# ipl-uw/ZeDO-Release

Hardware: AMD Instinct MI355X
Metric: poses/sec (1000-step sampler, H=50) (higher is better)
Workload: dtype f32; 1 GPU; BASELINE configs[2] (3DPW pw3d_test, H=50, 1000 steps): N=1015 poses/GPU x H=50 hypotheses, IPO 500 it (17 joints) + 1000 OIL steps + P1/P2 min-over-hypotheses selection; random-init ScoreModelFC_Adv weights, synthetic detections; settings=pw3d, rows_per_gpu=50750, poses_total=1015

## Files before the change

zedo-release_amd/csrc/zedo_gemm.hip:

```cpp
#include "zedo_internal.h"
#include "zedo_tile.h"

#include <atomic>
#include <cstdlib>

#ifdef ZEDO_UBENCH
#include "../../tools/ubench/zedo_tile_hooks.inc"
#else
#define TL_MARK(var)
#define TL_FLUSH(t0, t1, t2)
#endif

namespace zedo {

template <int BM, int BN, int WM, int WN, int EPI, int NBUF = 2, int BK = 32, int SCHED = 0, int KSKIP = 0, int KQ = 1>
__device__ __forceinline__ void layer_tile(const LayerArgs &a, const int m0, const int n0, const int out_m0) {
    constexpr int NW = WM * WN;
    constexpr int CPR = BK / 4;
    constexpr int RPD = 64 / CPR;
    constexpr int KG = BK / 8;
    static_assert(BK == 32 || BK == 16, "BK");
    constexpr int TM = BM / WM, TN = BN / WN;
    constexpr int TJ = TM / 32, TI = TN / 32;
    constexpr int IA = BN / RPD / NW, IB = BM / RPD / NW;
    constexpr int IPW = IA + IB;
    static_assert(TM % 32 == 0 && TN % 32 == 0 && IA >= 1 && IB >= 1 && (BN / RPD) % NW == 0 && (BM / RPD) % NW == 0, "tile");
    static_assert(NBUF >= 2 && (NBUF - 1) * IPW <= 63, "ring depth vs the 6-bit vmcnt");

    extern __shared__ __attribute__((aligned(16))) float smem[];
    float *As = smem;
    float *Bs = smem + NBUF * BN * BK;
    float *Ps = smem + layer_tile_lds(BM, BN, WM, NBUF, BK) / sizeof(float) - 3 * BN;

    const int tid = threadIdx.x;
    const int lane = tid & 63;
    const int wid = __builtin_amdgcn_readfirstlane(tid >> 6);
    const int wm = wid / WN, wn = wid % WN;
    const int li = lane & 31, kh = lane >> 5;

    const int drow = lane / CPR, dpos = lane % CPR;
    const int dswz = (BK == 32) ? (drow & 7) : ((drow >> 2) & 3);
    const char *Wbase = reinterpret_cast<const char *>(a.W + (size_t)(n0 + wid * IA * RPD) * a.ldw);
    const char *Xbase = reinterpret_cast<const char *>(a.X + (size_t)(m0 + wid * IB * RPD) * a.ldx);
    const unsigned wlane = (unsigned)(drow * a.ldw + (dpos ^ dswz) * 4) * 4u;
    const unsigned xlane = (unsigned)(drow * a.ldx + (dpos ^ dswz) * 4) * 4u;
    const unsigned lds0 = (unsigned)(size_t)(__attribute__((address_space(3))) float *)smem;
    auto dma_one = [&](int kt, int buf, int p) {
        if (p < IA)
            dma16(Wbase + (size_t)kt * (BK * 4) + (size_t)p * (RPD * 4) * a.ldw, wlane,
                  lds0 + (unsigned)(((buf * BN + (wid * IA + p) * RPD) * BK) * 4));
        else
            dma16(Xbase + (size_t)kt * (BK * 4) + (size_t)(p - IA) * (RPD * 4) * a.ldx, xlane,
                  lds0 + (unsigned)(((NBUF * BN + buf * BM + (wid * IB + (p - IA)) * RPD) * BK) * 4));
    };
    auto dma = [&](int kt, int buf) {
#pragma unroll
        for (int p = 0; p < IPW; ++p) dma_one(kt, buf, p);
    };

    const int fswz = (BK == 32) ? (li & 7) : ((li >> 2) & 3);
    int foff[KG];
#pragma unroll
    for (int kg = 0; kg < KG; ++kg) foff[kg] = ((2 * kg + kh) ^ fswz) * 4;
    const float *Ab0 = As + (wn * TN + li) * BK;
    const float *Bb0 = Bs + (wm * TM + li) * BK;
    f32x4 fa0[TI], fb0[TJ], fa1[TI], fb1[TJ];
    auto fread = [&](f32x4(&fa)[TI], f32x4(&fb)[TJ], int buf, int kg) {
#pragma unroll
        for (int i = 0; i < TI; ++i) fa[i] = *reinterpret_cast<const f32x4 *>(Ab0 + (buf * BN + i * 32) * BK + foff[kg]);
#pragma unroll
        for (int j = 0; j < TJ; ++j) fb[j] = *reinterpret_cast<const f32x4 *>(Bb0 + (buf * BM + j * 32) * BK + foff[kg]);
    };
    f32x16 acc[TI][TJ];
#pragma unroll
    for (int i = 0; i < TI; ++i)
#pragma unroll
        for (int j = 0; j < TJ; ++j)
#pragma unroll
            for (int e = 0; e < 16; ++e) acc[i][j][e] = 0.0f;
    auto mma = [&](const f32x4(&fa)[TI], const f32x4(&fb)[TJ]) {
#pragma unroll
        for (int e = 0; e < 4; ++e)
#pragma unroll
            for (int i = 0; i < TI; ++i)
#pragma unroll
                for (int j = 0; j < TJ; ++j)
                    acc[i][j] = __builtin_amdgcn_mfma_f32_32x32x2f32(fa[i][e], fb[j][e], acc[i][j], 0, 0, 0);
    };
    constexpr int H1 = (IPW + 1) / 2, H2 = IPW - H1;
    auto mma_dma = [&](const f32x4(&fa)[TI], const f32x4(&fb)[TJ], int kt, int buf, int p0, int cnt) {
#pragma unroll
        for (int e = 0; e < 4; ++e) {
#pragma unroll
            for (int q = 0; q < 4; ++q)
                if (q < cnt && q * 4 / cnt == e) {
                    dma_one(kt, buf, p0 + q);
                    __builtin_amdgcn_sched_barrier(0);
                }
#pragma unroll
            for (int i = 0; i < TI; ++i)
#pragma unroll
                for (int j = 0; j < TJ; ++j)
                    acc[i][j] = __builtin_amdgcn_mfma_f32_32x32x2f32(fa[i][e], fb[j][e], acc[i][j], 0, 0, 0);
            __builtin_amdgcn_sched_barrier(0);
        }
    };
    static_assert(SCHED >= 0 && SCHED <= 3, "SCHED: bit 0 = pinned reads, bit 1 = spread DMA");
    static_assert(!(SCHED & 2) || H1 <= 4, "spread DMA: at most 4 instructions per MFMA group");

    TL_MARK(tl0)
    if (EPI != EPI_PARTIAL && tid < BN / 4) {
        *reinterpret_cast<f32x4 *>(Ps + tid * 4) = *reinterpret_cast<const f32x4 *>(a.bias + n0 + tid * 4);
        if constexpr (EPI == EPI_GN_SILU || EPI == EPI_GN_SILU_RES) {
            *reinterpret_cast<f32x4 *>(Ps + BN + tid * 4) = *reinterpret_cast<const f32x4 *>(a.gamma + n0 + tid * 4);
            *reinterpret_cast<f32x4 *>(Ps + 2 * BN + tid * 4) = *reinterpret_cast<const f32x4 *>(a.beta + n0 + tid * 4);
        }
    }
    const int KT = a.K / BK;
    f32x16 qsum[KQ > 1 ? TI : 1][KQ > 1 ? TJ : 1];
    const int KTQ = KT / KQ;
#pragma unroll
    for (int t = 0; t < NBUF; ++t) dma(min(t, KT - 1), t);
    asm volatile("s_waitcnt vmcnt(%0)" ::"n"((NBUF - 1) * IPW) : "memory");
    __syncthreads();
    fread(fa0, fb0, 0, 0);
    TL_MARK(tl1)
    for (int kt0 = 0; kt0 < KT; kt0 += NBUF) {
#pragma unroll
      for (int buf = 0; buf < NBUF; ++buf) {
        const int kt = kt0 + buf;
        const int nxt = (buf + 1 == NBUF) ? 0 : buf + 1;
        const int prv = (buf == 0) ? NBUF - 1 : buf - 1;
        fread(fa1, fb1, buf, 1);
        if constexpr (SCHED & 1) __builtin_amdgcn_sched_barrier(0);
        if constexpr (SCHED & 2) mma_dma(fa0, fb0, min(kt - 1 + NBUF, KT - 1), prv, H1, H2);
        else mma(fa0, fb0);
        if constexpr (KG == 4) {
            fread(fa0, fb0, buf, 2);
            if constexpr (SCHED & 1) __builtin_amdgcn_sched_barrier(0);
            mma(fa1, fb1);
            if constexpr (SCHED & 1) __builtin_amdgcn_sched_barrier(0);
            fread(fa1, fb1, buf, 3);
            if constexpr (SCHED & 1) __builtin_amdgcn_sched_barrier(0);
            mma(fa0, fb0);
        }
        const bool skip_last = KSKIP == 1 && KG == 4 && buf == NBUF - 1;
        asm volatile("s_waitcnt vmcnt(%0)" ::"n"((NBUF - 2) * IPW) : "memory");
        __syncthreads();
        if (skip_last) {
        } else if constexpr (SCHED & 2) {
            fread(fa0, fb0, nxt, 0);
            __builtin_amdgcn_sched_barrier(0);
            mma_dma(fa1, fb1, min(kt + NBUF, KT - 1), buf, 0, H1);
        } else {
            dma(min(kt + NBUF, KT - 1), buf);
            fread(fa0, fb0, nxt, 0);
            if constexpr (SCHED & 1) __builtin_amdgcn_sched_barrier(0);
            mma(fa1, fb1);
            if constexpr (SCHED & 1) __builtin_amdgcn_sched_barrier(0);
        }
      }
      if constexpr (KQ > 1) {
          if ((kt0 + NBUF) % KTQ == 0) {
              const bool first = (kt0 + NBUF == KTQ);
#pragma unroll
              for (int i = 0; i < TI; ++i)
#pragma unroll
                  for (int j = 0; j < TJ; ++j)
#pragma unroll
                      for (int e = 0; e < 16; ++e) {
                          qsum[i][j][e] = first ? acc[i][j][e] : qsum[i][j][e] + acc[i][j][e];
                          acc[i][j][e] = 0.0f;
                      }
          }
      }
    }
    if constexpr (KQ > 1) {
#pragma unroll
        for (int i = 0; i < TI; ++i)
#pragma unroll
            for (int j = 0; j < TJ; ++j) acc[i][j] = qsum[i][j];
    }
    asm volatile("s_waitcnt vmcnt(0)" ::: "memory");
    __syncthreads();
    TL_MARK(tl2)

    {
        constexpr int NT = NW * 64;
        constexpr int SR = WM * 32;
        constexpr int CPRW = BN / 4;
        constexpr int RPI = 64 / CPRW;
        static_assert(CPRW <= 64 && 64 % CPRW == 0 && SR % (RPI * NW) == 0 && (SR * CPRW) % NT == 0, "stage shape");
        constexpr bool HAS_RES = (EPI == EPI_GN_SILU_RES || EPI == EPI_SDE);
        float *S = smem;
        float *obase = a.out + (size_t)out_m0 * a.ldo + n0;
#pragma unroll
        for (int j = 0; j < TJ; ++j) {
            if constexpr (HAS_RES) {
                constexpr int NI = SR / RPI / NW;
#pragma unroll
                for (int p = 0; p < NI; ++p) {
                    const int idx = wid * NI + p;
                    const int sr = idx * RPI + lane / CPRW, pos = lane % CPRW;
                    const int grow = (sr >> 5) * TM + j * 32 + (sr & 31);
                    __builtin_amdgcn_global_load_lds(
                        (const __attribute__((address_space(1))) void *)(reinterpret_cast<const char *>(obase) +
                                                                         ((unsigned)grow * (unsigned)a.ldo + (unsigned)((pos ^ (sr & 7)) * 4)) * 4u),
                        (__attribute__((address_space(3))) void *)(S + idx * RPI * BN), 16, 0, 0);
                }
                asm volatile("s_waitcnt vmcnt(0)" ::: "memory");
                __syncthreads();
            }
#pragma unroll
            for (int i = 0; i < TI; ++i) {
                float o[16];
                f32x4 b4[4], ga[4], be[4];
                const float *pc = Ps + wn * TN + i * 32 + 4 * kh;
#pragma unroll
                for (int g = 0; g < 4; ++g) {
                    b4[g] = *reinterpret_cast<const f32x4 *>(pc + 8 * g);
                    if constexpr (EPI == EPI_GN_SILU || EPI == EPI_GN_SILU_RES) {
                        ga[g] = *reinterpret_cast<const f32x4 *>(pc + BN + 8 * g);
                        be[g] = *reinterpret_cast<const f32x4 *>(pc + 2 * BN + 8 * g);
                    }
                }
                epilogue_values<EPI>(acc[i][j], b4, ga, be, a.sde_c, o);
                float *srow = S + (wm * 32 + li) * BN;
#pragma unroll
                for (int g = 0; g < 4; ++g) {
                    const int c = (wn * TN + i * 32 + 8 * g + 4 * kh) >> 2;
                    f32x4 *slot = reinterpret_cast<f32x4 *>(srow + ((c ^ (li & 7)) << 2));
                    f32x4 v = {o[4 * g], o[4 * g + 1], o[4 * g + 2], o[4 * g + 3]};
                    if constexpr (EPI == EPI_GN_SILU_RES) {
                        const f32x4 h = *slot;
#pragma unroll
                        for (int e = 0; e < 4; ++e) v[e] += h[e];
                    } else if constexpr (EPI == EPI_SDE) {
                        const f32x4 x = *slot;
#pragma unroll
                        for (int e = 0; e < 4; ++e) v[e] = __builtin_fmaf(a.sde_a, x[e], v[e]);
                    }
                    *slot = v;
                }
            }
            __syncthreads();
            if constexpr (EPI == EPI_SDE && BN == XLD) {
                if (a.rp.geom != nullptr) {
                    if (tid < SR) {
                        const int sr = tid;
                        const int b = m0 + (sr >> 5) * TM + j * 32 + (sr & 31);
                        if (b < a.rp.B) ZEDO_REPROJ_STAGED_ROW(17, S + sr * BN, sr & 7, b, a.rp);
                    }
                    __syncthreads();
                }
            }
#pragma unroll
            for (int pass = 0; pass < SR * CPRW / NT; ++pass) {
                const int qi = pass * NT + tid;
                const int sr = qi / CPRW, c = qi % CPRW;
                const f32x4 v = *reinterpret_cast<const f32x4 *>(S + sr * BN + ((c ^ (sr & 7)) << 2));
                const int grow = (sr >> 5) * TM + j * 32 + (sr & 31);
                const unsigned off = ((unsigned)grow * (unsigned)a.ldo + (unsigned)(c * 4)) * 4u;
                *reinterpret_cast<f32x4 *>(reinterpret_cast<char *>(obase) + off) = v;
            }
            if (j + 1 < TJ) __syncthreads();
        }
    }
    TL_FLUSH(tl0, tl1, tl2)
}

template <int BM, int BN, int WM, int WN, int EPI, int NBUF = 2, int BK = 32, int SCHED = 0, int KSKIP = 0, int KQ = 1>
__device__ __forceinline__ void layer_body(const LayerArgs &a, const int bid, const int nwg) {
    const int lid = xcd_tile(bid, nwg);
    const int ncol = a.N / BN;
    if constexpr (EPI == EPI_PARTIAL) {
        LayerArgs b = a;
        const int tile = lid >> 2, q = lid & 3;
        b.X = a.X + (size_t)q * a.K;
        b.W = a.W + (size_t)q * a.K;
        layer_tile<BM, BN, WM, WN, EPI, NBUF, BK, SCHED, KSKIP, 1>(b, tile * BM, 0, lid * BM);
        return;
    }
    layer_tile<BM, BN, WM, WN, EPI, NBUF, BK, SCHED, KSKIP, KQ>(a, (lid / ncol) * BM, (lid % ncol) * BN, (lid / ncol) * BM);
}

template <int BM, int BN, int WM, int WN, int EPI, int NBUF = 2, int BK = 32, int SCHED = 0, int WPE = 1, int KSKIP = 0, int KQ = 1>
__global__ __launch_bounds__(WM *WN * 64, WPE) void layer_kernel(LayerArgs a) {
    layer_body<BM, BN, WM, WN, EPI, NBUF, BK, SCHED, KSKIP, KQ>(a, blockIdx.x, gridDim.x);
}

constexpr int SCHED_BIG = 3, SCHED_SMALL = 0, SCHED_THIN = 3, SCHED_BK16 = 1;

constexpr int PAIR_BK = 16, PLAIN_WGS = 3, PLAIN_WPE = 2;
template <int EPI, int W8>
__global__ __launch_bounds__(W8 ? 512 : 256, W8 ? 6 : PLAIN_WGS) void layer_pair_kernel(LayerArgs big, LayerArgs small, int nbig) {
    const ClockProbe probe(big.clk != nullptr && blockIdx.x == 0 && threadIdx.x == 0);
    if constexpr (W8) {
        if ((int)blockIdx.x < nbig) layer_body<128, 128, 2, 4, EPI, 2, PAIR_BK, SCHED_BK16>(big, blockIdx.x, nbig);
        else layer_body<64, 128, 2, 4, EPI, 2, 32, SCHED_SMALL>(small, (int)blockIdx.x - nbig, (int)gridDim.x - nbig);
    } else {
        if ((int)blockIdx.x < nbig) layer_body<128, 128, 2, 2, EPI, 2, PAIR_BK, SCHED_BK16>(big, blockIdx.x, nbig);
        else layer_body<64, 64, 2, 2, EPI, 2, 32, SCHED_SMALL>(small, (int)blockIdx.x - nbig, (int)gridDim.x - nbig);
    }
    probe.stop(big.clk);
}


template <int EPI, int W8>
static hipError_t launch_pair(const LayerArgs &big, const LayerArgs &small, hipStream_t st) {
    constexpr int SM = 64, SN = W8 ? 128 : 64;
    constexpr size_t lds_big = layer_tile_lds(128, 128, 2, 2, PAIR_BK), lds_small = layer_tile_lds(SM, SN, 2, 2, 32);
    constexpr size_t lds = lds_big > lds_small ? lds_big : lds_small;
    if (big.Mp % 128 || small.Mp % SM || big.N % 128 || big.K % 64) return hipErrorInvalidValue;
    auto kern = layer_pair_kernel<EPI, W8>;
    static std::atomic<bool> attr_done[MAX_DEVICES];
    if (hipError_t e = allow_lds(reinterpret_cast<const void *>(kern), lds, attr_done); e != hipSuccess) return e;
    const int nbig = (big.Mp / 128) * (big.N / 128), nsmall = (small.Mp / SM) * (small.N / SN);
    hipLaunchKernelGGL(kern, dim3(nbig + nsmall), dim3(W8 ? 512 : 256), lds, st, big, small, nbig);
    return hipGetLastError();
}

template <int BM, int BN, int WM, int WN, int EPI, int NBUF = 2, int BK = 32, int SCHED = 0, int WPE = 1, int KSKIP = 0, int KQ = 1>
static hipError_t launch_cfg(const LayerArgs &a, hipStream_t st) {
    constexpr size_t lds = layer_tile_lds(BM, BN, WM, NBUF, BK);
    if (a.Mp <= 0 || a.Mp % BM || a.N % BN || a.K % (BK * NBUF * KQ)) return hipErrorInvalidValue;
    if (KSKIP && a.K != BK * NBUF) return hipErrorInvalidValue;
    auto kern = layer_kernel<BM, BN, WM, WN, EPI, NBUF, BK, SCHED, WPE, KSKIP, KQ>;
    static std::atomic<bool> attr_done[MAX_DEVICES];
    if (hipError_t e = allow_lds(reinterpret_cast<const void *>(kern), lds, attr_done); e != hipSuccess) return e;
    const int nwg = (a.Mp / BM) * (a.N / BN) * (EPI == EPI_PARTIAL ? 4 : 1);
    hipLaunchKernelGGL(kern, dim3(nwg), dim3(WM * WN * 64), lds, st, a);
    return hipGetLastError();
}

static LayerArgs rows_of(const LayerArgs &a, int row0, int rows) {
    LayerArgs b = a;
    b.X = a.X + (size_t)row0 * a.ldx;
    b.out = a.out + (size_t)row0 * a.ldo;
    b.Mp = rows;
    return b;
}

template <int EPI>
static hipError_t launch_small(const LayerArgs &a, hipStream_t st) {
    const int ncol = a.N / 128, cus = num_cus();
    if (a.Mp % 64 == 0 && (a.Mp / 64) * (a.N / 64) <= cus)
        return launch_cfg<64, 64, 2, 2, EPI, 4, 32, SCHED_THIN & 1>(a, st);
    if (a.Mp % 32 == 0 && (a.Mp / 32) * ncol <= cus) return launch_cfg<32, 128, 1, 4, EPI, 4, 32, SCHED_THIN & 1>(a, st);
    auto cost = [&](int bm, int slots_per_cu, double tile_us) {
        if (a.Mp % bm) return 1e30;
        const long tiles = (long)(a.Mp / bm) * ncol;
        const long rounds = (tiles + (long)cus * slots_per_cu - 1) / ((long)cus * slots_per_cu);
        return rounds * 6.0 + (double)((tiles + cus - 1) / cus) * tile_us;
    };
    const double kdepth = a.K / 1024.0;
    const double c32 = cost(32, 3, 14.5 * kdepth), c64 = cost(64, 3, 28.2 * kdepth), c128 = cost(128, 2, 55.1 * kdepth);
    if (c32 <= c64 && c32 <= c128) return launch_cfg<32, 128, 1, 4, EPI, 2, 32, SCHED_THIN>(a, st);
    if (c64 <= c128) return launch_cfg<64, 128, 2, 4, EPI, 2, 32, SCHED_THIN>(a, st);
    return launch_cfg<128, 128, 2, 2, EPI, 2, 32, SCHED_BIG, PLAIN_WPE>(a, st);
}

template <int EPI>
static hipError_t launch_wide(const LayerArgs &a, hipStream_t st) {
    if (a.K <= 64) {
        if (a.K == 64 && a.kzero8) return launch_cfg<64, 128, 2, 4, EPI, 2, 32, SCHED_THIN, 1, 1>(a, st);
        return launch_cfg<64, 128, 2, 4, EPI, 2, 32, SCHED_THIN>(a, st);
    }
    constexpr int WG_PER_CU = 3;
    constexpr int W8 = (EPI == EPI_GN_SILU_RES) ? 1 : 0;
    const int per_round = num_cus() * WG_PER_CU * 128 / (a.N / 128);
    int rows_big = (a.Mp / per_round) * per_round;
    if (rows_big == 0) {
        const int one_each = num_cus() * 128 / (a.N / 128);
        const int mix_big = (a.Mp / one_each) * one_each;
        constexpr int SMR = (W8 ? 64 : 32);
        if (mix_big > 0 && a.Mp > mix_big && (a.Mp - mix_big) % SMR == 0) {
            const double kd = a.K / 1024.0;
            const long small_tiles = (long)((a.Mp - mix_big) / SMR) * (a.N / 128);
            const double est_mix = (mix_big / one_each) * 55.1 * kd + (double)((small_tiles + num_cus() - 1) / num_cus()) * (W8 ? 28.2 : 13.9) * kd + 6.0;
            auto single = [&](int bm, int slots, double t) {
                if (a.Mp % bm) return 1e30;
                const long tiles = (long)(a.Mp / bm) * (a.N / 128);
                return (double)((tiles + (long)num_cus() * slots - 1) / ((long)num_cus() * slots)) * 6.0 + (double)((tiles + num_cus() - 1) / num_cus()) * t * kd;
            };
            const double est_single = fmin(fmin(single(32, 3, 14.5), single(64, 3, 28.2)), single(128, 2, 55.1));
            if (est_mix < est_single) rows_big = mix_big;
        }
    }
    const int rows_small = a.Mp - rows_big;
    if (rows_small > 0 && rows_big > 0) {
        if (W8 && rows_small >= 1536) return launch_pair<EPI, W8>(rows_of(a, 0, rows_big), rows_of(a, rows_big, rows_small), st);
        return launch_pair<EPI, 0>(rows_of(a, 0, rows_big), rows_of(a, rows_big, rows_small), st);
    }
    if (rows_big > 0) return launch_pair<EPI, W8>(rows_of(a, 0, rows_big), rows_of(a, rows_big, 0), st);
    return launch_small<EPI>(a, st);
}

hipError_t launch_layer(const LayerArgs &a, int epilogue, hipStream_t st) {
    if (a.N == XLD) {
        if (epilogue != EPI_SDE && epilogue != EPI_BIAS) return hipErrorInvalidValue;
        if (a.K % (4 * 32 * 4)) return hipErrorInvalidValue;
        if (a.Mp <= POST_SPLIT_ROWS && a.Mp % 32 == 0 && a.scratch) {
            LayerArgs p = a;
            p.K = a.K / 4; p.out = a.scratch; p.ldo = XLD;
            if (hipError_t e = launch_cfg<32, 64, 1, 2, EPI_PARTIAL, 4, 32, SCHED_THIN>(p, st); e != hipSuccess) return e;
            const bool sde = epilogue == EPI_SDE;
            return launch_post_reduce(sde ? a.out : nullptr, a.scratch, a.bias, a.sde_a, a.sde_c, sde ? 1 : 0, sde ? nullptr : a.out,
                                      sde ? a.rp : ReprojArgs{}, a.Mp, st);
        }
        const bool small = a.Mp <= 8192 && a.Mp % 32 == 0;
        switch (epilogue) {
            case EPI_SDE: return small ? launch_cfg<32, 64, 1, 2, EPI_SDE, 4, 32, SCHED_THIN, 1, 0, 4>(a, st) : launch_cfg<64, 64, 2, 2, EPI_SDE, 4, 32, SCHED_THIN, 1, 0, 4>(a, st);
            case EPI_BIAS: return small ? launch_cfg<32, 64, 1, 2, EPI_BIAS, 4, 32, SCHED_THIN, 1, 0, 4>(a, st) : launch_cfg<64, 64, 2, 2, EPI_BIAS, 4, 32, SCHED_THIN, 1, 0, 4>(a, st);
        }
        return hipErrorInvalidValue;
    }
    if (a.N % 128) return hipErrorInvalidValue;
    switch (epilogue) {
        case EPI_GN_SILU: return launch_wide<EPI_GN_SILU>(a, st);
        case EPI_GN_SILU_RES: return launch_wide<EPI_GN_SILU_RES>(a, st);
        case EPI_BIAS: return launch_wide<EPI_BIAS>(a, st);
        case EPI_BIAS_SILU: return launch_wide<EPI_BIAS_SILU>(a, st);
    }
    return hipErrorInvalidValue;
}

__global__ __launch_bounds__(256) void mfma_probe_kernel(float *out, int iters, long long *clk) {
    f32x16 acc[4];
    for (int i = 0; i < 4; ++i) for (int e = 0; e < 16; ++e) acc[i][e] = 0.f;
    const float a = threadIdx.x * 1e-3f, b = blockIdx.x * 1e-3f + 1.0f;
    long long t0 = 0, w0 = 0;
    if (threadIdx.x == 0 && blockIdx.x == 0) { t0 = clock64(); w0 = wall_clock64(); }
    for (int it = 0; it < iters; ++it) {
#pragma unroll
        for (int u = 0; u < 4; ++u)
#pragma unroll
            for (int i = 0; i < 4; ++i) acc[i] = __builtin_amdgcn_mfma_f32_32x32x2f32(a, b, acc[i], 0, 0, 0);
    }
    if (threadIdx.x == 0 && blockIdx.x == 0) { clk[0] = clock64() - t0; clk[1] = wall_clock64() - w0; }
    float s = 0;
    for (int i = 0; i < 4; ++i) for (int e = 0; e < 16; ++e) s += acc[i][e];
    out[blockIdx.x * 256 + threadIdx.x] = s;
}

__global__ __launch_bounds__(256) void mfma16_probe_kernel(float *out, int iters, long long *clk) {
    f32x16 acc[4];
    for (int i = 0; i < 4; ++i) for (int e = 0; e < 16; ++e) acc[i][e] = 0.f;
    f16x8 fa[4], fb[4];
    unsigned h = (threadIdx.x * 2654435761u) ^ (blockIdx.x * 40503u + 17u);
    for (int i = 0; i < 4; ++i)
        for (int e = 0; e < 8; ++e) {
            h = h * 1664525u + 1013904223u; fa[i][e] = (_Float16)(((int)(h >> 20) - 2048) * (1.0f / 4096.0f));
            h = h * 1664525u + 1013904223u; fb[i][e] = (_Float16)(((int)(h >> 20) - 2048) * (1.0f / 4096.0f));
        }
    long long t0 = 0, w0 = 0;
    if (threadIdx.x == 0 && blockIdx.x == 0) { t0 = clock64(); w0 = wall_clock64(); }
    for (int it = 0; it < iters; ++it) {
#pragma unroll
        for (int u = 0; u < 4; ++u) {
            const int s0 = (u & 1) * 2;
            acc[0] = __builtin_amdgcn_mfma_f32_32x32x16_f16(fa[s0], fb[s0], acc[0], 0, 0, 0);
            acc[1] = __builtin_amdgcn_mfma_f32_32x32x16_f16(fa[s0], fb[s0 + 1], acc[1], 0, 0, 0);
            acc[2] = __builtin_amdgcn_mfma_f32_32x32x16_f16(fa[s0 + 1], fb[s0], acc[2], 0, 0, 0);
            acc[3] = __builtin_amdgcn_mfma_f32_32x32x16_f16(fa[s0 + 1], fb[s0 + 1], acc[3], 0, 0, 0);
        }
    }
    if (threadIdx.x == 0 && blockIdx.x == 0) { clk[0] = clock64() - t0; clk[1] = wall_clock64() - w0; }
    float s = 0;
    for (int i = 0; i < 4; ++i) for (int e = 0; e < 16; ++e) s += acc[i][e];
    out[blockIdx.x * 256 + threadIdx.x] = s;
}

hipError_t probe_mfma_peak(int iters, double *tflops, double *shader_ghz, hipStream_t st, bool f16) {
    const int blocks = num_cus() * 2;
    float *d_out = nullptr;
    long long *d_clk = nullptr, clk[2] = {0, 0};
    hipEvent_t e0 = nullptr, e1 = nullptr;
    float ms = 0.f;
    hipError_t e = hipMalloc(&d_out, (size_t)blocks * 256 * sizeof(float));
    if (e == hipSuccess) e = hipMalloc(&d_clk, 16);
    if (e == hipSuccess) e = hipEventCreate(&e0);
    if (e == hipSuccess) e = hipEventCreate(&e1);
    if (e == hipSuccess) {
        if (f16) hipLaunchKernelGGL(mfma16_probe_kernel, dim3(blocks), dim3(256), 0, st, d_out, iters / 4, d_clk);
        else hipLaunchKernelGGL(mfma_probe_kernel, dim3(blocks), dim3(256), 0, st, d_out, iters / 4, d_clk);
        e = hipGetLastError();
    }
    if (e == hipSuccess) e = hipEventRecord(e0, st);
    if (e == hipSuccess) {
        if (f16) hipLaunchKernelGGL(mfma16_probe_kernel, dim3(blocks), dim3(256), 0, st, d_out, iters, d_clk);
        else hipLaunchKernelGGL(mfma_probe_kernel, dim3(blocks), dim3(256), 0, st, d_out, iters, d_clk);
        e = hipGetLastError();
    }
    if (e == hipSuccess) e = hipEventRecord(e1, st);
    if (e == hipSuccess) e = hipEventSynchronize(e1);
    if (e == hipSuccess) e = hipEventElapsedTime(&ms, e0, e1);
    if (e == hipSuccess) e = hipMemcpy(clk, d_clk, 16, hipMemcpyDeviceToHost);
    if (e == hipSuccess) {
        const double flop = (double)blocks * 4 * iters * 16 * 2.0 * 32 * 32 * (f16 ? 16 : 2);
        if (tflops) *tflops = flop / ms / 1e9;
        if (shader_ghz) *shader_ghz = clk[1] > 0 ? (double)clk[0] / ((double)clk[1] / 100e6) / 1e9 : 0.0;
    } else {
        (void)hipStreamSynchronize(st);
    }
    if (e0) (void)hipEventDestroy(e0);
    if (e1) (void)hipEventDestroy(e1);
    (void)hipFree(d_out);
    (void)hipFree(d_clk);
    return e;
}

#ifdef ZEDO_UBENCH
#include "../../tools/ubench/zedo_gemm_variants.inc"
#endif

}
```

Baseline: 321.2 poses/s.

## Choose GEMM tile split per shape with cached XCD-aware simulated scheduler

Replaces the hard-coded heuristic that splits wide-layer rows between big and small tile configurations with a planner. The planner starts from the old decision and, for mid-size row counts, simulates workgroup dispatch across XCDs and CU slots to try alternative single or paired tile splits. It keeps an alternative only if the estimated time improves by at least a margin. Plans are cached per shape to avoid host cost per launch. The risk is that the simulation model misjudges real kernel timing and picks a worse split for some shapes.

Measured after the change: 321.5 poses/s, median of 2. Within noise of the previous version (+0.1%).

```diff
diff --git a/zedo-release_amd/csrc/zedo_gemm.hip b/zedo-release_amd/csrc/zedo_gemm.hip
--- a/zedo-release_amd/csrc/zedo_gemm.hip
+++ b/zedo-release_amd/csrc/zedo_gemm.hip
@@ -1,4 +1,5 @@
 #include "zedo_internal.h"
+#include "zedo_plan.h"
 #include "zedo_tile.h"
 
 #include <atomic>
@@ -306,12 +307,30 @@
 }
 
 
+static LayerArgs rows_of(const LayerArgs &a, int row0, int rows) {
+    LayerArgs b = a;
+    b.X = a.X + (size_t)row0 * a.ldx;
+    b.out = a.out + (size_t)row0 * a.ldo;
+    b.Mp = rows;
+    return b;
+}
+
 template <int EPI, int W8>
-static hipError_t launch_pair(const LayerArgs &big, const LayerArgs &small, hipStream_t st) {
+static hipError_t launch_pair(const LayerArgs &a, const plan::Plan &p, hipStream_t st) {
     constexpr int SM = 64, SN = W8 ? 128 : 64;
     constexpr size_t lds_big = layer_tile_lds(128, 128, 2, 2, PAIR_BK), lds_small = layer_tile_lds(SM, SN, 2, 2, 32);
     constexpr size_t lds = lds_big > lds_small ? lds_big : lds_small;
-    if (big.Mp % 128 || small.Mp % SM || big.N % 128 || big.K % 64) return hipErrorInvalidValue;
+    LayerArgs big = rows_of(a, 0, 0), small = rows_of(a, a.Mp, 0);
+    int covered = 0;
+    for (int s = 0; s < p.nseg; ++s) {
+        const plan::Segment &g = p.seg[s];
+        if (g.row0 != covered || g.rows <= 0) return hipErrorInvalidValue;
+        if (g.bm == 128 && g.bn == 128 && s == 0) big = rows_of(a, g.row0, g.rows);
+        else if (g.bm == SM && g.bn == SN && s == p.nseg - 1) small = rows_of(a, g.row0, g.rows);
+        else return hipErrorInvalidValue;
+        covered += g.rows;
+    }
+    if (covered != a.Mp || big.Mp % 128 || small.Mp % SM || a.N % 128 || a.K % 64) return hipErrorInvalidValue;
     auto kern = layer_pair_kernel<EPI, W8>;
     static std::atomic<bool> attr_done[MAX_DEVICES];
     if (hipError_t e = allow_lds(reinterpret_cast<const void *>(kern), lds, attr_done); e != hipSuccess) return e;
@@ -333,31 +352,20 @@
     return hipGetLastError();
 }
 
-static LayerArgs rows_of(const LayerArgs &a, int row0, int rows) {
-    LayerArgs b = a;
-    b.X = a.X + (size_t)row0 * a.ldx;
-    b.out = a.out + (size_t)row0 * a.ldo;
-    b.Mp = rows;
-    return b;
-}
-
-template <int EPI>
-static hipError_t launch_small(const LayerArgs &a, hipStream_t st) {
-    const int ncol = a.N / 128, cus = num_cus();
-    if (a.Mp % 64 == 0 && (a.Mp / 64) * (a.N / 64) <= cus)
-        return launch_cfg<64, 64, 2, 2, EPI, 4, 32, SCHED_THIN & 1>(a, st);
-    if (a.Mp % 32 == 0 && (a.Mp / 32) * ncol <= cus) return launch_cfg<32, 128, 1, 4, EPI, 4, 32, SCHED_THIN & 1>(a, st);
-    auto cost = [&](int bm, int slots_per_cu, double tile_us) {
-        if (a.Mp % bm) return 1e30;
-        const long tiles = (long)(a.Mp / bm) * ncol;
-        const long rounds = (tiles + (long)cus * slots_per_cu - 1) / ((long)cus * slots_per_cu);
-        return rounds * 6.0 + (double)((tiles + cus - 1) / cus) * tile_us;
-    };
-    const double kdepth = a.K / 1024.0;
-    const double c32 = cost(32, 3, 14.5 * kdepth), c64 = cost(64, 3, 28.2 * kdepth), c128 = cost(128, 2, 55.1 * kdepth);
-    if (c32 <= c64 && c32 <= c128) return launch_cfg<32, 128, 1, 4, EPI, 2, 32, SCHED_THIN>(a, st);
-    if (c64 <= c128) return launch_cfg<64, 128, 2, 4, EPI, 2, 32, SCHED_THIN>(a, st);
-    return launch_cfg<128, 128, 2, 2, EPI, 2, 32, SCHED_BIG, PLAIN_WPE>(a, st);
+static const plan::Plan &cached_plan(int Mp, int N, int K, bool residual, int cus) {
+    struct Entry { int Mp, N, K, residual, cus; plan::Plan p; };
+    constexpr int SLOTS = 16;
+    thread_local Entry cache[SLOTS];
+    thread_local int used = 0, next = 0;
+    for (int i = 0; i < used; ++i) {
+        const Entry &e = cache[i];
+        if (e.Mp == Mp && e.N == N && e.K == K && e.residual == (int)residual && e.cus == cus) return e.p;
+    }
+    Entry &e = cache[next];
+    e = Entry{Mp, N, K, (int)residual, cus, plan::choose(Mp, N, K, residual, cus)};
+    next = (next + 1) % SLOTS;
+    if (used < SLOTS) ++used;
+    return e.p;
 }
 
 template <int EPI>
@@ -366,34 +374,22 @@
         if (a.K == 64 && a.kzero8) return launch_cfg<64, 128, 2, 4, EPI, 2, 32, SCHED_THIN, 1, 1>(a, st);
         return launch_cfg<64, 128, 2, 4, EPI, 2, 32, SCHED_THIN>(a, st);
     }
-    constexpr int WG_PER_CU = 3;
-    constexpr int W8 = (EPI == EPI_GN_SILU_RES) ? 1 : 0;
-    const int per_round = num_cus() * WG_PER_CU * 128 / (a.N / 128);
-    int rows_big = (a.Mp / per_round) * per_round;
-    if (rows_big == 0) {
-        const int one_each = num_cus() * 128 / (a.N / 128);
-        const int mix_big = (a.Mp / one_each) * one_each;
-        constexpr int SMR = (W8 ? 64 : 32);
-        if (mix_big > 0 && a.Mp > mix_big && (a.Mp - mix_big) % SMR == 0) {
-            const double kd = a.K / 1024.0;
-            const long small_tiles = (long)((a.Mp - mix_big) / SMR) * (a.N / 128);
-            const double est_mix = (mix_big / one_each) * 55.1 * kd + (double)((small_tiles + num_cus() - 1) / num_cus()) * (W8 ? 28.2 : 13.9) * kd + 6.0;
-            auto single = [&](int bm, int slots, double t) {
-                if (a.Mp % bm) return 1e30;
-                const long tiles = (long)(a.Mp / bm) * (a.N / 128);
-                return (double)((tiles + (long)num_cus() * slots - 1) / ((long)num_cus() * slots)) * 6.0 + (double)((tiles + num_cus() - 1) / num_cus()) * t * kd;
-            };
-            const double est_single = fmin(fmin(single(32, 3, 14.5), single(64, 3, 28.2)), single(128, 2, 55.1));
-            if (est_mix < est_single) rows_big = mix_big;
-        }
-    }
-    const int rows_small = a.Mp - rows_big;
-    if (rows_small > 0 && rows_big > 0) {
-        if (W8 && rows_small >= 1536) return launch_pair<EPI, W8>(rows_of(a, 0, rows_big), rows_of(a, rows_big, rows_small), st);
-        return launch_pair<EPI, 0>(rows_of(a, 0, rows_big), rows_of(a, rows_big, rows_small), st);
-    }
-    if (rows_big > 0) return launch_pair<EPI, W8>(rows_of(a, 0, rows_big), rows_of(a, rows_big, 0), st);
-    return launch_small<EPI>(a, st);
+    constexpr bool RES = (EPI == EPI_GN_SILU_RES);
+    if (a.Mp <= 0) return hipErrorInvalidValue;
+    const plan::Plan &p = cached_plan(a.Mp, a.N, a.K, RES, num_cus());
+    if (p.nseg == 0) return hipErrorInvalidValue;
+    switch (p.carrier) {
+        case plan::PAIR4: return launch_pair<EPI, 0>(a, p, st);
+        case plan::PAIR8:
+            if constexpr (RES) return launch_pair<EPI, 1>(a, p, st);
+            else return hipErrorInvalidValue;
+        case plan::SINGLE_64x64_R4: return launch_cfg<64, 64, 2, 2, EPI, 4, 32, SCHED_THIN & 1>(a, st);
+        case plan::SINGLE_32x128_R4: return launch_cfg<32, 128, 1, 4, EPI, 4, 32, SCHED_THIN & 1>(a, st);
+        case plan::SINGLE_32x128: return launch_cfg<32, 128, 1, 4, EPI, 2, 32, SCHED_THIN>(a, st);
+        case plan::SINGLE_64x128: return launch_cfg<64, 128, 2, 4, EPI, 2, 32, SCHED_THIN>(a, st);
+        case plan::SINGLE_128x128: return launch_cfg<128, 128, 2, 2, EPI, 2, 32, SCHED_BIG, PLAIN_WPE>(a, st);
+    }
+    return hipErrorInvalidValue;
 }
 
 hipError_t launch_layer(const LayerArgs &a, int epilogue, hipStream_t st) {
diff --git a/zedo-release_amd/csrc/zedo_plan.h b/zedo-release_amd/csrc/zedo_plan.h
--- /dev/null
+++ b/zedo-release_amd/csrc/zedo_plan.h
@@ -0,0 +1,235 @@
+#pragma once
+
+#include <cmath>
+#include <queue>
+#include <utility>
+#include <vector>
+
+namespace zedo {
+namespace plan {
+
+enum Carrier : int {
+    PAIR4 = 0,
+    PAIR8,
+    SINGLE_64x64_R4,
+    SINGLE_32x128_R4,
+    SINGLE_32x128,
+    SINGLE_64x128,
+    SINGLE_128x128,
+};
+
+struct Segment { int bm, bn, row0, rows; };
+
+struct Plan {
+    int carrier = SINGLE_128x128;
+    int nseg = 0;
+    Segment seg[3] = {};
+    int tiles(int s, int N) const { return (seg[s].rows / seg[s].bm) * (N / seg[s].bn); }
+    int grid(int N) const {
+        int g = 0;
+        for (int s = 0; s < nseg; ++s) g += tiles(s, N);
+        return g;
+    }
+    bool same(const Plan &o) const {
+        if (carrier != o.carrier || nseg != o.nseg) return false;
+        for (int s = 0; s < nseg; ++s)
+            if (seg[s].bm != o.seg[s].bm || seg[s].bn != o.seg[s].bn || seg[s].row0 != o.seg[s].row0 || seg[s].rows != o.seg[s].rows) return false;
+        return true;
+    }
+};
+
+constexpr int XCDS = 8;
+constexpr double OVERHEAD_US = 6.0;
+constexpr int PIN_BELOW = 2048, PIN_FROM = 24576;
+constexpr double MIN_GAIN = 0.01;
+
+inline double tile_us(int bm, int bn, int K) {
+    const double kd = K / 1024.0;
+    if (bm == 128) return 55.1 * kd;
+    if (bm == 64 && bn == 128) return 28.2 * kd;
+    if (bm == 64) return 13.9 * kd;
+    return 14.5 * kd;
+}
+inline int slots_per_cu(int carrier) { return carrier == SINGLE_128x128 ? 2 : 3; }
+
+inline Plan single(int carrier, int Mp) {
+    Plan p;
+    p.carrier = carrier;
+    const int bm = (carrier == SINGLE_128x128) ? 128 : (carrier == SINGLE_64x128 || carrier == SINGLE_64x64_R4) ? 64 : 32;
+    const int bn = (carrier == SINGLE_64x64_R4) ? 64 : 128;
+    if (Mp > 0 && Mp % bm == 0) {
+        p.nseg = 1;
+        p.seg[0] = Segment{bm, bn, 0, Mp};
+    }
+    return p;
+}
+inline Plan pair(int carrier, int Mp, int rows_big) {
+    Plan p;
+    p.carrier = carrier;
+    const int bn = (carrier == PAIR8) ? 128 : 64;
+    if (rows_big % 128 || (Mp - rows_big) % 64 || rows_big < 0 || rows_big > Mp) return p;
+    if (rows_big > 0) p.seg[p.nseg++] = Segment{128, 128, 0, rows_big};
+    if (Mp > rows_big) p.seg[p.nseg++] = Segment{64, bn, rows_big, Mp - rows_big};
+    return p;
+}
+
+inline double simulate_xcd(const int *cnt, const double *t, int nseg, int ncu, int slots) {
+    struct Cu { double now = 0.0; int n = 0; double rem[3] = {0, 0, 0}; };
+    if (ncu <= 0) return (cnt[0] + cnt[1] + cnt[2]) ? 1e30 : 0.0;
+    std::vector<Cu> cu(ncu);
+    int s = 0, left = nseg ? cnt[0] : 0;
+    auto next = [&]() -> double {
+        while (s < nseg && left == 0) { ++s; left = s < nseg ? cnt[s] : 0; }
+        if (s >= nseg) return -1.0;
+        --left;
+        return t[s];
+    };
+    auto due = [&](const Cu &c) {
+        double m = c.rem[0];
+        for (int i = 1; i < c.n; ++i) m = std::fmin(m, c.rem[i]);
+        return c.now + m * c.n;
+    };
+    bool more = true;
+    for (int r = 0; r < slots && more; ++r)
+        for (int c = 0; c < ncu && more; ++c) {
+            const double w = next();
+            if (w < 0) more = false;
+            else cu[c].rem[cu[c].n++] = w;
+        }
+    if (more) {
+        typedef std::pair<double, int> Ev;
+        std::priority_queue<Ev, std::vector<Ev>, std::greater<Ev>> q;
+        for (int c = 0; c < ncu; ++c) q.push(Ev(due(cu[c]), c));
+        std::vector<int> freed;
+        while (more && !q.empty()) {
+            const double now = q.top().first;
+            freed.clear();
+            while (!q.empty() && q.top().first <= now + 1e-9) {
+                Cu &c = cu[q.top().second];
+                freed.push_back(q.top().second);
+                q.pop();
+                const double each = (now - c.now) / c.n;
+                c.now = now;
+                int keep = 0;
+                for (int i = 0; i < c.n; ++i) {
+                    const double r = c.rem[i] - each;
+                    if (r > 1e-9) c.rem[keep++] = r;
+                }
+                c.n = keep;
+            }
+            while (more) {
+                int to = -1;
+                for (int c : freed)
+                    if (cu[c].n < slots && (to < 0 || cu[c].n < cu[to].n || (cu[c].n == cu[to].n && c < to))) to = c;
+                if (to < 0) break;
+                const double w = next();
+                if (w < 0) more = false;
+                else cu[to].rem[cu[to].n++] = w;
+            }
+            for (int c : freed)
+                if (cu[c].n > 0) q.push(Ev(due(cu[c]), c));
+        }
+    }
+    double end = 0.0;
+    for (const Cu &c : cu) {
+        double sum = c.now;
+        for (int i = 0; i < c.n; ++i) sum += c.rem[i];
+        end = std::fmax(end, sum);
+    }
+    return end;
+}
+
+inline double simulate(const Plan &p, int N, int K, int cus) {
+    if (p.nseg == 0 || cus <= 0) return 1e30;
+    const int slots = slots_per_cu(p.carrier);
+    double t[3] = {0, 0, 0};
+    for (int s = 0; s < p.nseg; ++s) t[s] = tile_us(p.seg[s].bm, p.seg[s].bn, K);
+    int seen[XCDS][4];
+    double seen_end[XCDS];
+    int nseen = 0;
+    double end = 0.0;
+    for (int x = 0; x < XCDS; ++x) {
+        int sig[4] = {cus / XCDS + (x < cus % XCDS ? 1 : 0), 0, 0, 0};
+        long first = 0;
+        for (int s = 0; s < p.nseg; ++s) {
+            const long last = first + p.tiles(s, N);
+            auto upto = [&](long b) { return b <= x ? 0L : (b - x + XCDS - 1) / XCDS; };
+            sig[1 + s] = (int)(upto(last) - upto(first));
+            first = last;
+        }
+        int hit = -1;
+        for (int i = 0; i < nseen && hit < 0; ++i)
+            if (seen[i][0] == sig[0] && seen[i][1] == sig[1] && seen[i][2] == sig[2] && seen[i][3] == sig[3]) hit = i;
+        if (hit < 0) {
+            for (int i = 0; i < 4; ++i) seen[nseen][i] = sig[i];
+            seen_end[nseen] = simulate_xcd(sig + 1, t, p.nseg, sig[0], slots);
+            hit = nseen++;
+        }
+        end = std::fmax(end, seen_end[hit]);
+    }
+    return end + OVERHEAD_US;
+}
+
+inline Plan legacy_plan(int Mp, int N, int K, bool residual, int cus) {
+    const int ncol = N / 128;
+    const double kd = K / 1024.0;
+    auto cost = [&](int bm, int slots, double tile) {
+        if (Mp % bm) return 1e30;
+        const long tiles = (long)(Mp / bm) * ncol;
+        const long rounds = (tiles + (long)cus * slots - 1) / ((long)cus * slots);
+        return rounds * 6.0 + (double)((tiles + cus - 1) / cus) * tile * kd;
+    };
+    const int per_round = cus * 3 * 128 / ncol;
+    int rows_big = (Mp / per_round) * per_round;
+    if (rows_big == 0) {
+        const int one_each = cus * 128 / ncol;
+        const int mix_big = (Mp / one_each) * one_each;
+        const int smr = residual ? 64 : 32;
+        if (mix_big > 0 && Mp > mix_big && (Mp - mix_big) % smr == 0) {
+            const long small_tiles = (long)((Mp - mix_big) / smr) * ncol;
+            const double est_mix = (mix_big / one_each) * 55.1 * kd + (double)((small_tiles + cus - 1) / cus) * (residual ? 28.2 : 13.9) * kd + 6.0;
+            const double est_single = std::fmin(std::fmin(cost(32, 3, 14.5), cost(64, 3, 28.2)), cost(128, 2, 55.1));
+            if (est_mix < est_single) rows_big = mix_big;
+        }
+    }
+    const int rows_small = Mp - rows_big;
+    if (rows_small > 0 && rows_big > 0) return pair(residual && rows_small >= 1536 ? PAIR8 : PAIR4, Mp, rows_big);
+    if (rows_big > 0) return pair(residual ? PAIR8 : PAIR4, Mp, rows_big);
+    if (Mp % 64 == 0 && (Mp / 64) * (N / 64) <= cus) return single(SINGLE_64x64_R4, Mp);
+    if (Mp % 32 == 0 && (Mp / 32) * ncol <= cus) return single(SINGLE_32x128_R4, Mp);
+    const double c32 = cost(32, 3, 14.5), c64 = cost(64, 3, 28.2), c128 = cost(128, 2, 55.1);
+    if (c32 <= c64 && c32 <= c128) return single(SINGLE_32x128, Mp);
+    if (c64 <= c128) return single(SINGLE_64x128, Mp);
+    return single(SINGLE_128x128, Mp);
+}
+
+inline Plan choose(int Mp, int N, int K, bool residual, int cus) {
+    Plan best = legacy_plan(Mp, N, K, residual, cus);
+    if (Mp <= PIN_BELOW || Mp >= PIN_FROM || best.nseg == 0 || best.carrier == SINGLE_64x64_R4 || best.carrier == SINGLE_32x128_R4)
+        return best;
+    double best_us = simulate(best, N, K, cus);
+    const double must_beat = best_us * (1.0 - MIN_GAIN);
+    auto offer = [&](const Plan &p) {
+        if (p.nseg == 0) return;
+        const double us = simulate(p, N, K, cus);
+        if (us < best_us - 1e-6 && us < must_beat) { best = p; best_us = us; }
+    };
+    const int ncol = N / 128;
+    const int one_each = cus * 128 / ncol, per_round = 3 * one_each;
+    const int rounds = Mp / per_round;
+    if (rounds == 0) {
+        offer(single(SINGLE_128x128, Mp));
+        offer(single(SINGLE_64x128, Mp));
+        offer(single(SINGLE_32x128, Mp));
+    }
+    for (int j = 0; j < 3; ++j) {
+        const int rows_big = rounds * per_round + j * one_each;
+        if (rows_big > Mp) break;
+        if (residual) offer(pair(PAIR8, Mp, rows_big));
+        offer(pair(PAIR4, Mp, rows_big));
+    }
+    return best;
+}
+
+}
+}
```
